# istellartech/OpenGoddard

Hardware: AMD Instinct MI355X
Metric: NLP-callback evals/sec (cost+constr+FD-Jacobian) (higher is better)
Workload: dtype f64; 1 GPU; polar_tsto: 2 phases, [6, 6] states, [3, 3] controls, [80, 80] LGL nodes; n=1442, m_eq=975, m_ineq=640, output_buffers=17 registered persistent-zero replicas of 18.6 MB in rotation, parallelism=fd-columns x1

## Files before the change

opengoddard_amd/csrc/ogk_kernels.hip:

```cpp
#include <hip/hip_runtime.h>
#include "ogk.h"
#include "og_dual.h"
#include OG_GEN_HEADER

typedef double v4f64 __attribute__((ext_vector_type(4)));

#ifndef OGK_EXP
#define OGK_EXP 0
#endif

#ifndef OGK_TRACE
#define OGK_TRACE 0
#endif

namespace {

struct XCol {
    typedef double scalar;
    const double* x0;
    int j;
    double xj;
    __device__ __forceinline__ double operator()(const int i) const {
        const double v = x0[i];
        return i == j ? xj : v;
    }
    __device__ __forceinline__ double ldy(const double* p) const { return *p; }
};

struct XColL {
    typedef double scalar;
    const double* x0;
    int j;
    double xj;
    const double* y0_first;
    const double* yl;
    __device__ __forceinline__ double operator()(const int i) const {
        const double v = x0[i];
        return i == j ? xj : v;
    }
    __device__ __forceinline__ double ldy(const double* p) const { return yl[(int)(p - y0_first)]; }
};

constexpr int TB_SLOTS = OgGen::N_TBLK > 0 ? OgGen::N_TBLK : 1;
struct XColT {
    typedef double scalar;
    const double* x0;
    int j;
    double xj;
    const double* tc;
    int qd[TB_SLOTS];
    double td[TB_SLOTS];
    __device__ __forceinline__ double operator()(const int i) const {
        const double v = x0[i];
        return i == j ? xj : v;
    }
    __device__ __forceinline__ double ldy(const double* p) const { return *p; }
    __device__ __forceinline__ const double* term_cache(const int tb) const {
        return (tc && qd[tb] != -2) ? tc + OgGen::TERM_OFF(tb) : nullptr;
    }
    __device__ __forceinline__ int term_q(const int tb) const { return qd[tb]; }
    __device__ __forceinline__ double term_v(const int tb) const { return td[tb]; }
};
__device__ __forceinline__ XColT make_xcolt(const ogk_args& a, const int j, const double xj, const double* tc) {
    XColT x;
    x.x0 = a.x0, x.j = j, x.xj = xj, x.tc = tc;
    const XCol plain{a.x0, j, xj};
#pragma unroll
    for (int tb = 0; tb < TB_SLOTS; ++tb) {
        x.qd[tb] = -1, x.td[tb] = 0.0;
        if (tc && tb < OgGen::N_TBLK && j >= 0) {
            x.qd[tb] = OgGen::sum_term_q(tb, j);
            if (x.qd[tb] >= 0) x.td[tb] = OgGen::sum_term(tb, x.qd[tb], plain, a.cvec);
        }
    }
    return x;
}
constexpr bool TERM_CACHE = OgGen::N_TERMS > 0 && OgGen::N_TERMS <= 2048;
constexpr int TERM_DOUBLES = TERM_CACHE ? OgGen::N_TERMS + 16 : 0;

template <int THREADS>
__device__ __forceinline__ void fill_terms(const ogk_args& a, double* tc) {
    struct XBase {
        typedef double scalar;
        const double* x0;
        __device__ __forceinline__ double operator()(const int i) const { return x0[i]; }
    };
    const XBase xb{a.x0};
#pragma unroll
    for (int tb = 0; tb < OgGen::N_TBLK; ++tb)
        for (int q = (int)threadIdx.x; q < OgGen::TERM_LEN(tb); q += THREADS)
            tc[OgGen::TERM_OFF(tb) + q] = OgGen::sum_term(tb, q, xb, a.cvec);
}

__device__ __forceinline__ bool jt_needs_fill(const ogk_args& a) {
    const unsigned st = *a.jt_state, gen = *a.jt_launches;
    return !a.jt_sparse | (st == gen - 1u);
}
__device__ __forceinline__ void jt_mark_nan_fill(const ogk_args& a) {
    if (a.jt_sparse) __hip_atomic_store(a.jt_state, *a.jt_launches, __ATOMIC_RELAXED, __HIP_MEMORY_SCOPE_AGENT);
}

constexpr int ROWS_COLS_PER_THREAD = 8;

__device__ __forceinline__ int defect_block_to_group(int bx, int* nt_out) {
    for (int g = 0; g < OgGen::N_GROUPS; ++g) {
        if (OgGen::G_KIND(g) != 1) continue;
        const int ntiles = (OgGen::G_LEN(g) + 15) >> 4;
        if (bx < ntiles) { *nt_out = bx; return g; }
        bx -= ntiles;
    }
    *nt_out = 0;
// ... 284 lines not shown
    const int NP = KS * 4;
    const int tid = (int)threadIdx.x;
    const int wave = tid >> 6, lane = tid & 63, lk = lane >> 4;

    double* dpanel = lds;
    double* xt = lds + KS * 64;
    double* ybuf = xt + OgGen::MAX_NMV * NP;
    const double* src = a.dfrag + a.dfrag_off[rec0.v[5]] + (long)nt * KS * 64;
    constexpr int UNR = 4;
    double pv[UNR];
#pragma unroll
    for (int u = 0; u < UNR; ++u)
        pv[u] = (tid + SWEEP_THREADS * u < KS * 64) ? src[tid + SWEEP_THREADS * u] : 0.0;
    const XCol base{a.x0, -1, 0.0};
    for (int s = wave; s < OgGen::MAX_NMV; s += SWEEP_WAVES)
        for (int l = lane; l < NP; l += 64) {
            double v = 0.0;
            if (s < nmv && l < N) {
                v = OgGen::mv_operand(mv0 + s, l, base, a.cvec);
                if (nt == 0) a.xop[OGT_SLOT[mv0 + s].v[4] + l] = v;
            }
            xt[s * NP + l] = v;
        }
#pragma unroll
    for (int u = 0; u < UNR; ++u)
        if (tid + SWEEP_THREADS * u < KS * 64) dpanel[tid + SWEEP_THREADS * u] = pv[u];
    for (int i = tid + SWEEP_THREADS * UNR; i < KS * 64; i += SWEEP_THREADS) dpanel[i] = src[i];
    __syncthreads();

    constexpr int TR = (OgGen::MAX_NMV + SWEEP_WAVES - 1) / SWEEP_WAVES;
    if (wave == SWEEP_WAVES - 1) {
        const int srow = lane & 15;
        v4f64 acc = {0.0, 0.0, 0.0, 0.0};
        const double* xrow = xt + (srow < OgGen::MAX_NMV ? srow : 0) * NP;
        const bool live = srow < nmv;
        constexpr int CH = 8;
        double bv[CH], av[CH];
#pragma unroll
        for (int u = 0; u < CH; ++u) {
            bv[u] = u < KS ? dpanel[u * 64 + lane] : 0.0;
            av[u] = (u < KS && live) ? xrow[u * 4 + lk] : 0.0;
        }
        for (int ks0 = 0; ks0 < KS; ks0 += CH) {
            double bn[CH], an[CH];
#pragma unroll
            for (int u = 0; u < CH; ++u) {
                const int ks = ks0 + CH + u;
                bn[u] = ks < KS ? dpanel[ks * 64 + lane] : 0.0;
                an[u] = (ks < KS && live) ? xrow[ks * 4 + lk] : 0.0;
            }
#pragma unroll
            for (int u = 0; u < CH; ++u)
                if (ks0 + u < KS) acc = __builtin_amdgcn_mfma_f64_16x16x4f64(av[u], bv[u], acc, 0, 0, 0);
#pragma unroll
            for (int u = 0; u < CH; ++u) { bv[u] = bn[u]; av[u] = an[u]; }
        }
#pragma unroll
        for (int reg = 0; reg < 4; ++reg) ybuf[(lk + 4 * reg) * 16 + (lane & 15)] = acc[reg];
    }
    const int k = nt * 16 + lane;
    const bool node_on = lane < 16 && k < N;
    double T[TR];
#pragma unroll
    for (int r = 0; r < TR; ++r) {
        const int s = wave + r * SWEEP_WAVES;
        T[r] = (node_on && s < nmv) ? OgGen::tail_one(mv0 + s, k, base, a.cvec) : 0.0;
    }
    __syncthreads();
    if (!node_on) return;
#pragma unroll
    for (int r = 0; r < TR; ++r) {
        const int s = wave + r * SWEEP_WAVES;
        if (s >= nmv) break;
        const ogt_int8 rec = OGT_SLOT[mv0 + s];
        const double y = ybuf[s * 16 + lane];
        const int row = rec.v[3] + k;
        publish_row<FUSED>(a, row, y - T[r]);
        a.t0[row] = T[r];
        a.y0[rec.v[4] + k] = y;
    }
}

template <bool FUSED>
__device__ __forceinline__ void eval_rows_body(const ogk_args& a, const int bx, double* lds) {
    bool terms = false;
    if (TERM_CACHE) {
#pragma unroll
        for (int u = 0; u < SWEEP_WAVES; ++u) {
            const int w2 = bx * SWEEP_WAVES + u;
            if (w2 < OGT_N_ROWWAVES) terms = terms || OGT_ROWWAVE[w2].w != 0;
        }
        if (terms) {
            fill_terms<SWEEP_THREADS>(a, lds);
            __syncthreads();
        }
    }
    const int w = bx * SWEEP_WAVES + ((int)threadIdx.x >> 6);
    if (w >= OGT_N_ROWWAVES) return;
    const int4 rw = OGT_ROWWAVE[w];
    const int k = rw.y + ((int)threadIdx.x & 63);
    if (k >= rw.z) return;
    const XColT base = make_xcolt(a, -1, 0.0, terms ? lds : nullptr);
    int row;
    const double v = OgGen::item_value(rw.x, 0, k, base, a.y0, a.cvec, &row);
    publish_row<FUSED>(a, row, v);
}

#ifdef OGK_HAS_MAIN
__global__ __launch_bounds__(SWEEP_THREADS) void ogk_eval(const ogk_args a, const int ndef) {
    extern __shared__ __attribute__((aligned(16))) double lds[];
    const int id = (int)blockIdx.x;
    if (id == 0 && threadIdx.x == 0) {
        *a.nonfinite_next = 0;
        if (a.jt_bump) __hip_atomic_store(a.jt_launches, *a.jt_launches + 1u, __ATOMIC_RELAXED, __HIP_MEMORY_SCOPE_AGENT);
    }
    if (id < ndef) eval_defect_body<false>(a, id, lds);
    else eval_rows_body<false>(a, id - ndef, lds);
}
#endif

#ifndef OGK_LIGHT_COLS
#define OGK_LIGHT_COLS 4
#endif
constexpr int LIGHT_COLS = OGK_LIGHT_COLS;
constexpr int HEAVY_FLAG = 1 << 30;

__device__ __forceinline__ bool marked(const unsigned* bits, const int r) {
    return (bits[r >> 5] >> (r & 31)) & 1u;
}

__device__ __forceinline__ void fill_row(const ogk_args& a, double* jrow, const unsigned* bits,
                                         const int own_lo, const int own_hi, const int first,
                                         const int stride, const bool all_finite,
                                         const bool z_from_this_launch = false) {
    if (OGK_EXP & 16) return;
    if (all_finite) {
        const int a0 = (int)((reinterpret_cast<unsigned long long>(jrow) >> 3) & 1);
        const double2 zero2 = make_double2(0.0, 0.0);
// ... 272 lines not shown
            atomicOr(&bits[r >> 5], 1u << (r & 31));
        }
        __syncthreads();
        fill_row(a, a.jt + (long)(j - a.col_lo) * OgGen::M, bits, own_lo, own_hi, tid, SWEEP_THREADS, false, true);
        __syncthreads();
    }
}

__device__ __forceinline__ void finish_eval(const ogk_args& a, const unsigned n_eval, unsigned* bits) {
    __shared__ int s_last;
    __builtin_amdgcn_s_waitcnt(0);
    __syncthreads();
    if (threadIdx.x == 0) {
        const unsigned t = __hip_atomic_fetch_add(a.ready, 1u, __ATOMIC_RELAXED, __HIP_MEMORY_SCOPE_AGENT);
        int last = 0;
        if (t + 1u == n_eval) {
            const int bad = __hip_atomic_load(a.nonfinite, __ATOMIC_RELAXED, __HIP_MEMORY_SCOPE_AGENT);
            const unsigned st = __hip_atomic_load(a.jt_state, __ATOMIC_RELAXED, __HIP_MEMORY_SCOPE_AGENT);
            const unsigned gen = __hip_atomic_load(a.jt_launches, __ATOMIC_RELAXED, __HIP_MEMORY_SCOPE_AGENT) + 1u;
            __hip_atomic_store(a.ready, 0u, __ATOMIC_RELAXED, __HIP_MEMORY_SCOPE_AGENT);
            __hip_atomic_store(a.jt_launches, gen, __ATOMIC_RELAXED, __HIP_MEMORY_SCOPE_AGENT);
            __hip_atomic_store(a.nonfinite_result, bad, __ATOMIC_RELAXED, __HIP_MEMORY_SCOPE_AGENT);
            if (a.ptail) a.ptail[OgGen::M] = (double)bad;
            __hip_atomic_store(a.nonfinite, 0, __ATOMIC_RELAXED, __HIP_MEMORY_SCOPE_AGENT);
            if (bad != 0) __hip_atomic_store(a.jt_state, gen, __ATOMIC_RELAXED, __HIP_MEMORY_SCOPE_AGENT);
            last = (bad != 0 || st == gen - 1u) ? 1 : 0;
        }
        s_last = last;
    }
    __syncthreads();
    if (s_last) fz_fill_from_z(a, bits);
}

template <class Store>
__device__ __forceinline__ void base_products_tile(const double* panel, const int N, const int nt,
                                                   const int nmv, const double* xt, const int xstride,
                                                   const Store& store) {
    const int lane = (int)threadIdx.x & 63, lk = lane >> 4, srow = lane & 15;
    const int KS = (N + 3) >> 2;
    const double* bsrc = panel + lane;
    const bool live = srow < nmv;
    const double* xrow = xt + (live ? srow : 0) * xstride;
    v4f64 acc = {0.0, 0.0, 0.0, 0.0};
    constexpr int CH = 8;
    double bv[CH], av[CH];
#pragma unroll
    for (int u = 0; u < CH; ++u) {
        const int l = u * 4 + lk;
        bv[u] = u < KS ? bsrc[u * 64] : 0.0;
        av[u] = (u < KS && live && l < N) ? xrow[l] : 0.0;
    }
    for (int ks0 = 0; ks0 < KS; ks0 += CH) {
        double bn[CH], an[CH];
#pragma unroll
        for (int u = 0; u < CH; ++u) {
            const int ks = ks0 + CH + u;
            const int l = ks * 4 + lk;
            bn[u] = ks < KS ? bsrc[ks * 64] : 0.0;
            an[u] = (ks < KS && live && l < N) ? xrow[l] : 0.0;
        }
#pragma unroll
        for (int u = 0; u < CH; ++u)
            if (ks0 + u < KS) acc = __builtin_amdgcn_mfma_f64_16x16x4f64(av[u], bv[u], acc, 0, 0, 0);
#pragma unroll
        for (int u = 0; u < CH; ++u) { bv[u] = bn[u]; av[u] = an[u]; }
    }
    const int k = nt * 16 + (lane & 15);
#pragma unroll
    for (int reg = 0; reg < 4; ++reg) {
        const int st = lk + 4 * reg;
        if (st < nmv && k < N) store(st, k, acc[reg]);
    }
}

constexpr int FZ_COLS = OGT_LGRP_COLS;
template <class XA>
__device__ __forceinline__ void eval_item_paired(const ogk_args& a, const int4 item, const XA& xa, const bool base_role,
                                                 const double dx, double* jrow, double* packed) {
    int row;
    const double v = OgGen::item_value(item.x, item.y, item.z, xa, a.y0, a.cvec, &row);
    const double v0 = __shfl_down(v, FZ_COLS);
    if (!base_role) {
        const double q = (v - v0) / dx;
        jrow[row] = q;
        if (packed) *packed = q;
    }
}

constexpr int FZ_MAXN = OgGen::MAX_NODES;
constexpr int FZ_NP = ((FZ_MAXN + 3) / 4) * 4;
constexpr int FZ_ROUNDS = 2;
constexpr int FZ_ITEM_WAVES = SWEEP_WAVES - 1;
constexpr size_t FZ_TILE_DOUBLES = (size_t)(FZ_NP / 4) * 64 + (size_t)OgGen::MAX_NMV * (FZ_NP + FZ_MAXN);
constexpr size_t FZ_LDS_BYTES = (FZ_TILE_DOUBLES + TERM_DOUBLES) * sizeof(double);

__device__ __forceinline__ void lds_flag_raise(int* flag, const int value) {
    __builtin_amdgcn_fence(__ATOMIC_RELEASE, "workgroup", "local");
    *reinterpret_cast<volatile int*>(flag) = value;
}
__device__ __forceinline__ int lds_flag_wait(int* flag) {
    int v;
    while ((v = *reinterpret_cast<volatile int*>(flag)) == 0) __builtin_amdgcn_s_sleep(1);
    __builtin_amdgcn_fence(__ATOMIC_ACQUIRE, "workgroup", "local");
    return v;
}

#if OGK_TRACE
#define FZ_TRACE_DECL(kind_) long long tr_[6] = {(long long)__builtin_amdgcn_s_memrealtime(), 0, 0, 0, 0, 0}; \
    const int tr_kind_ = (kind_)
#define FZ_STAMP(i) tr_[i] = (long long)__builtin_amdgcn_s_memrealtime()
#define FZ_TRACE_OUT(a_)                                                                                   \
    do {                                                                                                   \
        if (((int)threadIdx.x & 63) == 0 && (a_).trace) {                                                  \
            double* t_ = (a_).trace + ((long)blockIdx.x * SWEEP_WAVES + ((int)threadIdx.x >> 6)) * 8;       \
            t_[0] = (double)tr_kind_; t_[1] = (double)tr_[0]; t_[2] = (double)tr_[1]; t_[3] = (double)tr_[2]; \
            t_[4] = (double)tr_[3]; t_[5] = (double)tr_[4]; t_[6] = (double)tr_[5];                          \
            t_[7] = (double)__builtin_amdgcn_s_memrealtime();                                              \
        }                                                                                                  \
    } while (0)
#else
#define FZ_TRACE_DECL(kind_) do { } while (0)
#define FZ_STAMP(i) do { } while (0)
#define FZ_TRACE_OUT(a_) do { } while (0)
#endif

struct FzTile {
    double* dpanel;
    double* xt;
    double* yb;
};
__device__ __forceinline__ FzTile fz_tile_lds(double* lds) {
    FzTile t;
    t.dpanel = lds;
    t.xt = lds + (FZ_NP / 4) * 64;
    t.yb = t.xt + OgGen::MAX_NMV * FZ_NP;
    return t;
}
__device__ __forceinline__ void fz_stage_tile(const ogk_args& a, const FzTile& t, const int nt, const int mv0,
                                              const int nmv, const int N, const int phase) {
    const int tid = (int)threadIdx.x, lane = tid & 63, wave = tid >> 6;
    const int KS = (N + 3) >> 2, NP = KS << 2;
    constexpr int ST_D = (FZ_NP / 4 * 64 + SWEEP_THREADS - 1) / SWEEP_THREADS;
    constexpr int ST_S = (OgGen::MAX_NMV + SWEEP_WAVES - 1) / SWEEP_WAVES, ST_L = (FZ_NP + 63) / 64;
    const XCol xbase{a.x0, -1, 0.0};
    double st_d[ST_D];
    const double* src = a.dfrag + a.dfrag_off[phase] + (long)nt * KS * 64;
#pragma unroll
    for (int u = 0; u < ST_D; ++u) {
        const int i = tid + u * SWEEP_THREADS;
        st_d[u] = i < KS * 64 ? src[i] : 0.0;
    }
#pragma unroll
    for (int u = 0; u < ST_S; ++u)
#pragma unroll
        for (int q = 0; q < ST_L; ++q) {
            const int sl = wave + u * SWEEP_WAVES, l = lane + q * 64;
            if (sl < nmv && l < NP) t.xt[sl * NP + l] = l < N ? OgGen::mv_operand(mv0 + sl, l, xbase, a.cvec) : 0.0;
        }
#pragma unroll
    for (int u = 0; u < ST_D; ++u) {
        const int i = tid + u * SWEEP_THREADS;
        if (i < KS * 64) t.dpanel[i] = st_d[u];
    }
}

__device__ __forceinline__ void fz_light_body(const ogk_args& a, const int b, double* lds) {
    __shared__ int s_flag;
    FZ_TRACE_DECL(1);
    const ogt_int8 grp = OGT_LGRP[b];
    const int first_j = grp.v[0], cnt = grp.v[1], y0_first = grp.v[2], nt = grp.v[3];
    const int mv0 = grp.v[4], nmv = grp.v[5], N = grp.v[6], phase = grp.v[7] & 0xffff;
    const bool terms = TERM_CACHE && (grp.v[7] >> 16) != 0;
    double* tc = lds + FZ_TILE_DOUBLES;
    const bool has_tile = nmv > 0;
    const int tid = (int)threadIdx.x;
    const int lane = tid & 63, wave = tid >> 6;
    const bool service = wave == SWEEP_WAVES - 1;
    const int cl = lane % FZ_COLS;
    const bool base_role = lane >= FZ_COLS;
    const int ji = first_j + cl;
    const bool item_on = !service && lane < 2 * FZ_COLS && cl < cnt && ji >= a.col_lo && ji < a.col_hi;
    const int4 coli = OGT_LRNG[b * FZ_COLS + cl];
    const double xb = a.x0[item_on ? ji : first_j];
    const double hh = a.h[item_on ? ji : first_j];
    int4 item = make_int4(0, 0, 0, 0);
    const bool has_item = item_on && coli.x + wave < coli.y;
    if (has_item) item = OGT_ELEM[coli.x + wave];

    const FzTile t = fz_tile_lds(lds);
    if (tid == 0) s_flag = 0;
    if (has_tile && !(OGK_FZ & 4)) fz_stage_tile(a, t, nt, mv0, nmv, N, phase);
    if (terms) fill_terms<SWEEP_THREADS>(a, tc);
    lds_barrier();
    FZ_STAMP(1);
    if (service) {
        if (has_tile && !(OGK_FZ & 2))
            base_products_tile(t.dpanel, N, nt, nmv, t.xt, ((N + 3) >> 2) << 2,
                               [&](const int st, const int k, const double v) { t.yb[st * N + k] = v; });
        FZ_STAMP(2);
        if (lane == 0) lds_flag_raise(&s_flag, 1);
        FZ_TRACE_OUT(a);
        return;
    }
    if (has_item && !(OGK_FZ & 2048)) {
        const double xj = xb + hh;
        const double dx = xj - xb;
        double* jrow = a.jt + (long)(ji - a.col_lo) * OgGen::M;
        double* pcol = a.pvals ? a.pvals + a.poff[ji] + (coli.z - coli.x) : nullptr;
        const XColT xa = make_xcolt(a, base_role ? -1 : ji, xj, terms ? tc : nullptr);
        double tv[FZ_ROUNDS];
        int trow[FZ_ROUNDS], tyo[FZ_ROUNDS];
#pragma unroll
        for (int r = 0; r < FZ_ROUNDS; ++r) {
            const int e = coli.x + wave + r * FZ_ITEM_WAVES;
            tv[r] = 0.0, trow[r] = 0, tyo[r] = -1;
            if (e < coli.y) {
                const int4 it = r == 0 ? item : OGT_ELEM[e];
                tv[r] = OgGen::item_tail(it.x, it.y, it.z, xa, a.cvec, &trow[r], &tyo[r]);
            }
        }
        lds_flag_wait(&s_flag);
        FZ_STAMP(3);
#pragma unroll
        for (int r = 0; r < FZ_ROUNDS; ++r) {
            const double v = tyo[r] >= 0 ? t.yb[tyo[r] - y0_first] - tv[r] : tv[r];
            const double v0 = __shfl_down(v, FZ_COLS);
            const int e = coli.x + wave + r * FZ_ITEM_WAVES;
            if (!base_role && e < coli.y) {
                const double q = (v - v0) / dx;
                jrow[trow[r]] = q;
                if (pcol) pcol[e] = q;
            }
        }
        const XColL xl{a.x0, base_role ? -1 : ji, xj, a.y0 + y0_first, t.yb};
        for (int e = coli.x + wave + FZ_ROUNDS * FZ_ITEM_WAVES; e < coli.y; e += FZ_ITEM_WAVES)
            eval_item_paired(a, OGT_ELEM[e], xl, base_role, dx, jrow, pcol ? pcol + e : nullptr);
    }
    FZ_STAMP(4);
    FZ_TRACE_OUT(a);
}

__device__ __forceinline__ void fz_heavy_part(const ogk_args& a, const int pidx, double* lds) {
    __shared__ int s_flag;
    FZ_TRACE_DECL(2);
    const ogt_int8 rec = OGT_HPART[pidx];
    const int j = rec.v[0];
    if (j < a.col_lo || j >= a.col_hi) return;
    const int y0_first = rec.v[3], nt = rec.v[4], mv0 = rec.v[5], nmv = rec.v[6];
    const int N = rec.v[7] & 0xfffff, phase = (rec.v[7] >> 20) & 0x3ff;
    const bool terms = TERM_CACHE && ((rec.v[7] >> 30) & 1) != 0;
    double* tc = lds + FZ_TILE_DOUBLES;
    const bool has_tile = nmv > 0;
    const int tid = (int)threadIdx.x;
    const int lane = tid & 63, wave = tid >> 6;
    const bool service = wave == SWEEP_WAVES - 1;
    const double xb = a.x0[j];
    const double hh = a.h[j];
    const int il = lane & 31;
    const bool base_role = lane >= 32;
    int4 slot = make_int4(0, 0, 0, 0), item = make_int4(0, 0, 0, 0);
    const bool has_slot = !service && rec.v[1] + wave < rec.v[2];
    if (has_slot) {
        slot = OGT_HSLOT[rec.v[1] + wave];
        item = OGT_HELEM[slot.x + (il < slot.y ? il : 0)];
    }
    const FzTile t = fz_tile_lds(lds);
    if (tid == 0) s_flag = 0;
    if (has_tile) fz_stage_tile(a, t, nt, mv0, nmv, N, phase);
    if (terms) fill_terms<SWEEP_THREADS>(a, tc);
    lds_barrier();
    FZ_STAMP(1);
    if (service) {
        if (has_tile)
            base_products_tile(t.dpanel, N, nt, nmv, t.xt, ((N + 3) >> 2) << 2,
                               [&](const int st, const int k, const double v) { t.yb[st * N + k] = v; });
        FZ_STAMP(2);
        if (lane == 0) lds_flag_raise(&s_flag, 1);
        FZ_TRACE_OUT(a);
        return;
    }
    if (has_slot) {
        const double xj = xb + hh;
        const double dx = xj - xb;
        double* jrow = a.jt + (long)(j - a.col_lo) * OgGen::M;
        double* pcol = a.pvals ? a.pvals + a.poff[j] : nullptr;
        const XColT xa = make_xcolt(a, base_role ? -1 : j, xj, terms ? tc : nullptr);
        for (int s0 = rec.v[1] + wave; s0 < rec.v[2]; s0 += FZ_ROUNDS * FZ_ITEM_WAVES) {
            double tv[FZ_ROUNDS];
            int trow[FZ_ROUNDS], tyo[FZ_ROUNDS], cnt[FZ_ROUNDS], tpos[FZ_ROUNDS];
#pragma unroll
            for (int r = 0; r < FZ_ROUNDS; ++r) {
                const int s = s0 + r * FZ_ITEM_WAVES;
                tv[r] = 0.0, trow[r] = 0, tyo[r] = -1, cnt[r] = 0, tpos[r] = 0;
                if (s < rec.v[2]) {
                    const int4 sl = (r == 0 && s0 == rec.v[1] + wave) ? slot : OGT_HSLOT[s];
                    const int4 it = (r == 0 && s0 == rec.v[1] + wave) ? item : OGT_HELEM[sl.x + (il < sl.y ? il : 0)];
                    cnt[r] = sl.y;
                    tpos[r] = it.w;
                    tv[r] = OgGen::item_tail(it.x, it.y, it.z, xa, a.cvec, &trow[r], &tyo[r]);
                }
            }
            if (s0 == rec.v[1] + wave) {
                lds_flag_wait(&s_flag);
                FZ_STAMP(3);
            }
#pragma unroll
            for (int r = 0; r < FZ_ROUNDS; ++r) {
                const double v = tyo[r] >= 0 ? t.yb[tyo[r] - y0_first] - tv[r] : tv[r];
                const double v0 = __shfl_down(v, 32);
                if (!base_role && il < cnt[r]) {
                    const double q = (v - v0) / dx;
                    jrow[trow[r]] = q;
                    if (pcol) pcol[tpos[r]] = q;
                }
            }
        }
    }
    FZ_STAMP(4);
    FZ_TRACE_OUT(a);
}

__device__ __forceinline__ void fz_tile_body(const ogk_args& a, const int bx, double* lds) {
    __shared__ int s_flags[3];
    FZ_TRACE_DECL(3);
    const int4 tile = OGT_FTILE[bx];
    const int slot = tile.x, ct0 = tile.y, nt = tile.z, nct = tile.w;
    const ogt_int8 rec = OGT_SLOT[slot];
    const int N = rec.v[0], leaf = rec.v[2], row0 = rec.v[3];
    const bool diag = rec.v[6] & 1, generic = rec.v[6] & 2;
    const int dep0 = rec.v[7] >> 12, ndep = rec.v[7] & 0xfff;
    const int KS = (N + 3) >> 2;
    const int tid = (int)threadIdx.x;
    const int wave = tid >> 6, lane = tid & 63, lk = lane >> 4, kk = lane & 15;
    double* xt = lds;
    double* yb = lds + FZ_NP;
    double* tb = yb + 16;
    double* td = tb + 16;
    const XCol xbase{a.x0, -1, 0.0};
    for (int l = tid; l < KS * 4; l += SWEEP_THREADS)
        xt[l] = l < N ? OgGen::mv_operand(slot, l, xbase, a.cvec) : 0.0;
    if (tid < 3) s_flags[tid] = 0;
    const int k = nt * 16 + kk;
    const bool k_on = k < N;
    const double* bsrc = a.dfrag + a.dfrag_off[rec.v[5]] + (long)nt * KS * 64 + lane;
    constexpr int CH = 10;
    const int prod_wave = SWEEP_WAVES - 1;
    const int term_wave = nct < SWEEP_WAVES - 1 ? SWEEP_WAVES - 2 : SWEEP_WAVES - 1;
    const bool diag_here = diag && nt >= ct0 && nt < ct0 + nct;
    const int diag_wave = nct < SWEEP_WAVES - 2 ? SWEEP_WAVES - 3 : -1;
    const bool col_wave = wave < nct;
    double bv[CH];
    if (col_wave || wave == prod_wave) {
#pragma unroll
        for (int u = 0; u < CH; ++u) bv[u] = (u < KS) ? bsrc[u * 64] : 0.0;
    }
    lds_barrier();
    FZ_STAMP(1);
    if (!col_wave) {
        if (wave == diag_wave) {
            if (diag_here && lk == 0 && k_on && leaf + k >= a.col_lo && leaf + k < a.col_hi) {
                const int jd = leaf + k;
                const double xbd = a.x0[jd];
                const XCol xd{a.x0, jd, xbd + a.h[jd]};
                td[kk] = OgGen::tail_one(slot, k, xd, a.cvec);
            }
            if (lane == 0) lds_flag_raise(&s_flags[2], 1);
        }
        if (wave == term_wave && lk == 0) tb[kk] = k_on ? OgGen::tail_one(slot, k, xbase, a.cvec) : 0.0;
        if (wave == term_wave && lane == 0) lds_flag_raise(&s_flags[1], 1);
        if (wave == prod_wave) {
                v4f64 accb = {0.0, 0.0, 0.0, 0.0};
            for (int ks0 = 0; ks0 < KS; ks0 += CH) {
                double bn[CH];
#pragma unroll
                for (int u = 0; u < CH; ++u) {
                    const int ks = ks0 + CH + u;
                    bn[u] = (ks < KS) ? bsrc[ks * 64] : 0.0;
                }
#pragma unroll
                for (int u = 0; u < CH; ++u) {
                    const int ks = ks0 + u;
                    if (ks < KS) accb = __builtin_amdgcn_mfma_f64_16x16x4f64(xt[ks * 4 + lk], bv[u], accb, 0, 0, 0);
                }
#pragma unroll
                for (int u = 0; u < CH; ++u) bv[u] = bn[u];
            }
            if (lk == 0) yb[kk] = accb[0];
            FZ_STAMP(2);
            if (lane == 0) lds_flag_raise(&s_flags[0], 1);
        }
        FZ_TRACE_OUT(a);
        return;
    }
    const int l0 = (ct0 + wave) * 16;
    if (l0 >= N || leaf + l0 >= a.col_hi || leaf + l0 + 16 <= a.col_lo) return;
    const int la = l0 + kk;
    const bool a_on = la < N;
    const double xa_b = a.x0[a_on ? leaf + la : leaf];
    const double xa_h = a.h[a_on ? leaf + la : leaf];
    const int row = row0 + (k_on ? k : 0);
    double xbv[4], hv[4];
#pragma unroll
    for (int reg = 0; reg < 4; ++reg) {
        const int lc = l0 + lk + 4 * reg;
        const int jj = leaf + ((k_on && lc < N) ? lc : 0);
        xbv[reg] = a.x0[jj];
        hv[reg] = a.h[jj];
    }
    double t_diag = 0.0;
    bool have_diag = false;
    {
        const int lc = k;
        const int reg = (lc - l0 - lk) >> 2;
        have_diag = diag && k_on && lc >= l0 + lk && ((lc - l0 - lk) & 3) == 0 && reg < 4 && lc < N &&
                    leaf + lc >= a.col_lo && leaf + lc < a.col_hi;
        if (have_diag && diag_wave < 0) {
            const int jd = leaf + lc;
            const double xbd = a.x0[jd];
            const XCol xd{a.x0, jd, xbd + a.h[jd]};
            t_diag = OgGen::tail_one(slot, k, xd, a.cvec);
        }
    }
    double hit_v = 0.0;
    if (a_on) {
        const XCol xa{a.x0, leaf + la, xa_b + xa_h};
        hit_v = OgGen::mv_operand(slot, la, xa, a.cvec);
    }
    v4f64 acc = {0.0, 0.0, 0.0, 0.0};
    for (int ks0 = 0; ks0 < KS; ks0 += CH) {
        double bn[CH];
#pragma unroll
        for (int u = 0; u < CH; ++u) {
            const int ks = ks0 + CH + u;
            bn[u] = (ks < KS) ? bsrc[ks * 64] : 0.0;
        }
#pragma unroll
        for (int u = 0; u < CH; ++u) {
            const int ks = ks0 + u;
            if (ks < KS) {
                const double aop = (ks * 4 + lk == la) ? hit_v : xt[ks * 4 + lk];
                acc = __builtin_amdgcn_mfma_f64_16x16x4f64(aop, bv[u], acc, 0, 0, 0);
            }
        }
#pragma unroll
        for (int u = 0; u < CH; ++u) bv[u] = bn[u];
    }
    FZ_STAMP(2);
    lds_flag_wait(&s_flags[1]);
    lds_flag_wait(&s_flags[0]);
    if (diag_wave >= 0 && l0 == nt * 16) {
        lds_flag_wait(&s_flags[2]);
        if (have_diag) t_diag = td[kk];
    }
    FZ_STAMP(3);
    if (!k_on) return;
    const double t_base = tb[kk];
    const double f_base = yb[kk] - t_base;
#pragma unroll
    for (int reg = 0; reg < 4; ++reg) {
        const int lc = l0 + lk + 4 * reg;
        const int j = leaf + lc;
        if (lc >= N || j < a.col_lo || j >= a.col_hi) continue;
        const double xj = xbv[reg] + hv[reg];
        const double dx = xj - xbv[reg];
        double t = (have_diag && lc == k) ? t_diag : t_base;
        if (generic) {
            bool reads = diag && k == lc;
            for (int d = dep0; d < dep0 + ndep; ++d) {
                const int kind = OgGen::DEP_KIND(d), base_d = OgGen::DEP_BASE(d);
                reads = reads || (kind == 1 ? (base_d + k == j)
                                            : (j >= base_d && j < base_d + OgGen::DEP_CNT(d)));
            }
            if (reads) {
                const XCol xg{a.x0, j, xj};
                t = OgGen::tail_one(slot, k, xg, a.cvec);
            }
        }
        const double val = acc[reg] - t;
        const double q = (val - f_base) / dx;
        a.jt[(long)(j - a.col_lo) * OgGen::M + row] = q;
        if (a.pvals) a.pvals[a.poff[j] + k] = q;
    }
    FZ_STAMP(4);
    FZ_TRACE_OUT(a);
}

#ifndef OGK_FUSED_ATTR
#define OGK_FUSED_ATTR __attribute__((amdgpu_waves_per_eu(4)))
#endif
#ifdef OGK_HAS_FUSED
__global__ __launch_bounds__(SWEEP_THREADS) OGK_FUSED_ATTR void ogk_fused(const ogk_args a, const int ndef, const int n_eval,
                                                           const int group_lo, const int n_light, const int sum_lo,
                                                           const int n_sum) {
    extern __shared__ __attribute__((aligned(16))) double lds[];
    int id = (int)blockIdx.x;
    if (id < n_eval) {
        FZ_TRACE_DECL(0);
        if (!(OGK_FZ & 16)) {
            if (id < ndef) eval_defect_body<true>(a, id, lds);
            else eval_rows_body<true>(a, id - ndef, lds);
        }
        FZ_STAMP(1);
        finish_eval(a, (unsigned)n_eval, reinterpret_cast<unsigned*>(lds));
        FZ_STAMP(4);
        FZ_TRACE_OUT(a);
        return;
    }
    id -= n_eval;
#ifndef OGK_ORDER
#define OGK_ORDER 0
#endif
    const int n_tile = OGT_N_FTILES, n_heavy = OGT_N_HPART;
    int kind, idx;
    if (OGK_ORDER == 0) {
        if (id < n_light) kind = 0, idx = id;
        else if (id < n_light + n_heavy) kind = 1, idx = id - n_light;
        else kind = 2, idx = id - n_light - n_heavy;
// ... 247 lines not shown
```

opengoddard_amd/codegen.py:

```python
from __future__ import annotations

import hashlib

import numpy as np

from . import trace as _tr

import os

HEAVY_COLUMN_ELEMENTS = 32
LIGHT_COLS = 4


def fused_cols(n):
    env = os.environ.get("OG_FUSED_COLS")
    return int(env) if env else 16


def tile_cols():
    env = os.environ.get("OG_TILE_COLS")
    return max(1, min(7, int(env))) if env else 7


MAX_GROUP_OUTPUTS = int(os.environ.get("OG_MAX_GROUP_OUTPUTS", "1"))
# ... 1031 lines not shown
          ",\n".join("    {{%s}}" % ", ".join(str(int(v)) for v in r) for r in (lgrp or [[0] * 8])),
          "};"]
    L += table("int4", "OGT_HSLOT", hslot)
    L += table("int4", "OGT_HELEM", helem)
    L += table("int4", "OGT_LRNG", lrng)
    L += ["static constexpr int OGT_N_LGRP = %d;" % len(light_groups),
          "static const int OGH_LGRP_J[%d] = {%s};" % (len(light_groups) + 1, ", ".join(
              [str(r[0]) for r in light_groups] + [str(P.n)]))]
    with_sum = [i for i, r in enumerate(lgrp) if r[7] & (1 << 16)]
    without = [i for i, r in enumerate(lgrp) if not r[7] & (1 << 16)]
    L += ["static __device__ const int OGT_LSUM[%d] = {%s};" % (max(len(with_sum), 1), ", ".join(map(str, with_sum or [0]))),
          "static __device__ const int OGT_LPLAIN[%d] = {%s};" % (max(len(without), 1), ", ".join(map(str, without or [0]))),
          "static const unsigned char OGH_LGRP_SUM[%d] = {%s};" % (max(len(lgrp), 1), ", ".join(
              "1" if r[7] & (1 << 16) else "0" for r in (lgrp or [[0] * 8])))]
    L += table("int4", "OGT_ROWWAVE", rowwaves)
    L.append("static constexpr int OGT_N_ROWWAVES = %d;" % len(rowwaves))
    L += table("int4", "OGT_COL", col)
    L += table("int4", "OGT_ELEM", elem)
    L += table("int4", "OGT_TILE", tiles)
    ftiles = []
    for si, sl in enumerate(P.mv):
        t16 = (sl.length + 15) // 16
        ngrp = -(-t16 // tile_cols())
        per = -(-t16 // ngrp)
        for c0 in range(0, t16, per):
            for nt in range(t16):
                ftiles.append([si, c0, nt, min(per, t16 - c0)])
    L += table("int4", "OGT_FTILE", ftiles)
    L.append("static constexpr int OGT_N_FTILES = %d;" % len(ftiles))
    L += table("ogt_int8", "OGT_SLOT", [[r] for r in []] or None) if False else \
        ["static __device__ const ogt_int8 OGT_SLOT[%d] = {" % max(len(slots), 1),
         ",\n".join("    {{%s}}" % ", ".join(str(int(v)) for v in r) for r in (slots or [[0] * 8])),
         "};"]
    L += ["static constexpr int OGT_N_TILES = %d;" % len(tiles),
          "static __device__ const int OGT_HEAVY[%d] = {%s};" % (
              max(len(heavy), 1), ", ".join(str(j) for j in heavy) or "0"),
          "#endif", ""]
    return L


def program_hash(source):
    return hashlib.sha256(source.encode()).hexdigest()[:16]
```

Before: 678.9 million callback evals/s.

## Route item tail evaluation through a shared noinline call and pipeline item loops

Item and slot tail evaluations now go through one out-of-line function (item_tail_at, __noinline__ by default) instead of being inlined at every call site via tail_one/item_value. The intent is to shrink code size and register pressure in the fused kernels. The item loops in the two fused column paths are rewritten as a software pipeline: each iteration computes the current tail, prefetches the next element descriptor, and then finishes the previous one. The wait on the staged y tile is deferred until a value that reads y is actually consumed. The risk is call overhead, since ABI register save/restore can slow the hot per-item path. A trace stamp macro is also added.

```diff
diff --git a/opengoddard_amd/csrc/ogk_kernels.hip b/opengoddard_amd/csrc/ogk_kernels.hip
--- a/opengoddard_amd/csrc/ogk_kernels.hip
+++ b/opengoddard_amd/csrc/ogk_kernels.hip
@@ -25,20 +25,6 @@
         return i == j ? xj : v;
     }
     __device__ __forceinline__ double ldy(const double* p) const { return *p; }
-};
-
-struct XColL {
-    typedef double scalar;
-    const double* x0;
-    int j;
-    double xj;
-    const double* y0_first;
-    const double* yl;
-    __device__ __forceinline__ double operator()(const int i) const {
-        const double v = x0[i];
-        return i == j ? xj : v;
-    }
-    __device__ __forceinline__ double ldy(const double* p) const { return yl[(int)(p - y0_first)]; }
 };
 
 constexpr int TB_SLOTS = OgGen::N_TBLK > 0 ? OgGen::N_TBLK : 1;
@@ -77,6 +63,39 @@
 }
 constexpr bool TERM_CACHE = OgGen::N_TERMS > 0 && OgGen::N_TERMS <= 2048;
 constexpr int TERM_DOUBLES = TERM_CACHE ? OgGen::N_TERMS + 16 : 0;
+
+#ifndef OGK_ITEM_CALL
+#define OGK_ITEM_CALL 1
+#endif
+#if OGK_ITEM_CALL
+#define OGK_ITEM_FN __device__ __noinline__
+#else
+#define OGK_ITEM_FN __device__ __forceinline__
+#endif
+struct ItemTail {
+    double v;
+    int row;
+    int yoff;
+};
+OGK_ITEM_FN ItemTail item_tail_at(const int g, const int o, const int k, const double* x0, const int j, const double xj,
+                                  const double* cv) {
+    const XCol x{x0, j, xj};
+    ItemTail r;
+    r.v = OgGen::item_tail(g, o, k, x, cv, &r.row, &r.yoff);
+    return r;
+}
+__device__ __forceinline__ ItemTail item_tail_of(const int4 it, const XColT& x, const double* cv) {
+    if (TERM_CACHE && x.tc) {
+        ItemTail r;
+        r.v = OgGen::item_tail(it.x, it.y, it.z, x, cv, &r.row, &r.yoff);
+        return r;
+    }
+    return item_tail_at(it.x, it.y, it.z, x.x0, x.j, x.xj, cv);
+}
+__device__ __forceinline__ double slot_tail_at(const int slot, const int g, const int k, const double* x0, const int j,
+                                               const double xj, const double* cv) {
+    return item_tail_at(g, slot - OgGen::G_MV0(g), k, x0, j, xj, cv).v;
+}
 
 template <int THREADS>
 __device__ __forceinline__ void fill_terms(const ogk_args& a, double* tc) {
@@ -459,7 +478,7 @@
 #pragma unroll
     for (int r = 0; r < TR; ++r) {
         const int s = wave + r * SWEEP_WAVES;
-        T[r] = (node_on && s < nmv) ? OgGen::tail_one(mv0 + s, k, base, a.cvec) : 0.0;
+        T[r] = (node_on && s < nmv) ? slot_tail_at(mv0 + s, blk.x, k, a.x0, -1, 0.0, a.cvec) : 0.0;
     }
     __syncthreads();
     if (!node_on) return;
@@ -496,9 +515,8 @@
     const int k = rw.y + ((int)threadIdx.x & 63);
     if (k >= rw.z) return;
     const XColT base = make_xcolt(a, -1, 0.0, terms ? lds : nullptr);
-    int row;
-    const double v = OgGen::item_value(rw.x, 0, k, base, a.y0, a.cvec, &row);
-    publish_row<FUSED>(a, row, v);
+    const ItemTail it = item_tail_of(make_int4(rw.x, 0, k, 0), base, a.cvec);
+    publish_row<FUSED>(a, it.row, it.yoff >= 0 ? a.y0[it.yoff] - it.v : it.v);
 }
 
 #ifdef OGK_HAS_MAIN
@@ -879,22 +897,8 @@
 }
 
 constexpr int FZ_COLS = OGT_LGRP_COLS;
-template <class XA>
-__device__ __forceinline__ void eval_item_paired(const ogk_args& a, const int4 item, const XA& xa, const bool base_role,
-                                                 const double dx, double* jrow, double* packed) {
-    int row;
-    const double v = OgGen::item_value(item.x, item.y, item.z, xa, a.y0, a.cvec, &row);
-    const double v0 = __shfl_down(v, FZ_COLS);
-    if (!base_role) {
-        const double q = (v - v0) / dx;
-        jrow[row] = q;
-        if (packed) *packed = q;
-    }
-}
-
 constexpr int FZ_MAXN = OgGen::MAX_NODES;
 constexpr int FZ_NP = ((FZ_MAXN + 3) / 4) * 4;
-constexpr int FZ_ROUNDS = 2;
 constexpr int FZ_ITEM_WAVES = SWEEP_WAVES - 1;
 constexpr size_t FZ_TILE_DOUBLES = (size_t)(FZ_NP / 4) * 64 + (size_t)OgGen::MAX_NMV * (FZ_NP + FZ_MAXN);
 constexpr size_t FZ_LDS_BYTES = (FZ_TILE_DOUBLES + TERM_DOUBLES) * sizeof(double);
@@ -914,6 +918,7 @@
 #define FZ_TRACE_DECL(kind_) long long tr_[6] = {(long long)__builtin_amdgcn_s_memrealtime(), 0, 0, 0, 0, 0}; \
     const int tr_kind_ = (kind_)
 #define FZ_STAMP(i) tr_[i] = (long long)__builtin_amdgcn_s_memrealtime()
+#define FZ_STAMP_LANDED(v) do { asm volatile("" :: "v"(v)); FZ_STAMP(5); } while (0)
 #define FZ_TRACE_OUT(a_)                                                                                   \
     do {                                                                                                   \
         if (((int)threadIdx.x & 63) == 0 && (a_).trace) {                                                  \
@@ -926,6 +931,7 @@
 #else
 #define FZ_TRACE_DECL(kind_) do { } while (0)
 #define FZ_STAMP(i) do { } while (0)
+#define FZ_STAMP_LANDED(v) do { } while (0)
 #define FZ_TRACE_OUT(a_) do { } while (0)
 #endif
 
@@ -991,6 +997,7 @@
     int4 item = make_int4(0, 0, 0, 0);
     const bool has_item = item_on && coli.x + wave < coli.y;
     if (has_item) item = OGT_ELEM[coli.x + wave];
+    FZ_STAMP_LANDED(grp.v[0] + coli.x + item.x);
 
     const FzTile t = fz_tile_lds(lds);
     if (tid == 0) s_flag = 0;
@@ -1013,33 +1020,31 @@
         double* jrow = a.jt + (long)(ji - a.col_lo) * OgGen::M;
         double* pcol = a.pvals ? a.pvals + a.poff[ji] + (coli.z - coli.x) : nullptr;
         const XColT xa = make_xcolt(a, base_role ? -1 : ji, xj, terms ? tc : nullptr);
-        double tv[FZ_ROUNDS];
-        int trow[FZ_ROUNDS], tyo[FZ_ROUNDS];
-#pragma unroll
-        for (int r = 0; r < FZ_ROUNDS; ++r) {
-            const int e = coli.x + wave + r * FZ_ITEM_WAVES;
-            tv[r] = 0.0, trow[r] = 0, tyo[r] = -1;
-            if (e < coli.y) {
-                const int4 it = r == 0 ? item : OGT_ELEM[e];
-                tv[r] = OgGen::item_tail(it.x, it.y, it.z, xa, a.cvec, &trow[r], &tyo[r]);
-            }
-        }
-        lds_flag_wait(&s_flag);
-        FZ_STAMP(3);
-#pragma unroll
-        for (int r = 0; r < FZ_ROUNDS; ++r) {
-            const double v = tyo[r] >= 0 ? t.yb[tyo[r] - y0_first] - tv[r] : tv[r];
-            const double v0 = __shfl_down(v, FZ_COLS);
-            const int e = coli.x + wave + r * FZ_ITEM_WAVES;
-            if (!base_role && e < coli.y) {
-                const double q = (v - v0) / dx;
-                jrow[trow[r]] = q;
-                if (pcol) pcol[e] = q;
-            }
-        }
-        const XColL xl{a.x0, base_role ? -1 : ji, xj, a.y0 + y0_first, t.yb};
-        for (int e = coli.x + wave + FZ_ROUNDS * FZ_ITEM_WAVES; e < coli.y; e += FZ_ITEM_WAVES)
-            eval_item_paired(a, OGT_ELEM[e], xl, base_role, dx, jrow, pcol ? pcol + e : nullptr);
+        ItemTail prev = {0.0, 0, -1};
+        bool seen = false;
+        int4 it = item;
+        for (int e = coli.x + wave; ; e += FZ_ITEM_WAVES) {
+            const bool more = e < coli.y;
+            ItemTail cur = {0.0, 0, -1};
+            if (more) cur = item_tail_of(it, xa, a.cvec);
+            if (e + FZ_ITEM_WAVES < coli.y) it = OGT_ELEM[e + FZ_ITEM_WAVES];
+            if (e != coli.x + wave) {
+                if (prev.yoff >= 0 && !seen) {
+                    lds_flag_wait(&s_flag);
+                    seen = true;
+                    FZ_STAMP(3);
+                }
+                const double v = prev.yoff >= 0 ? t.yb[prev.yoff - y0_first] - prev.v : prev.v;
+                const double v0 = __shfl_down(v, FZ_COLS);
+                if (!base_role) {
+                    const double q = (v - v0) / dx;
+                    jrow[prev.row] = q;
+                    if (pcol) pcol[e - FZ_ITEM_WAVES] = q;
+                }
+            }
+            if (!more) break;
+            prev = cur;
+        }
     }
     FZ_STAMP(4);
     FZ_TRACE_OUT(a);
@@ -1069,6 +1074,7 @@
         slot = OGT_HSLOT[rec.v[1] + wave];
         item = OGT_HELEM[slot.x + (il < slot.y ? il : 0)];
     }
+    FZ_STAMP_LANDED(rec.v[0] + slot.x + item.x);
     const FzTile t = fz_tile_lds(lds);
     if (tid == 0) s_flag = 0;
     if (has_tile) fz_stage_tile(a, t, nt, mv0, nmv, N, phase);
@@ -1090,35 +1096,40 @@
         double* jrow = a.jt + (long)(j - a.col_lo) * OgGen::M;
         double* pcol = a.pvals ? a.pvals + a.poff[j] : nullptr;
         const XColT xa = make_xcolt(a, base_role ? -1 : j, xj, terms ? tc : nullptr);
-        for (int s0 = rec.v[1] + wave; s0 < rec.v[2]; s0 += FZ_ROUNDS * FZ_ITEM_WAVES) {
-            double tv[FZ_ROUNDS];
-            int trow[FZ_ROUNDS], tyo[FZ_ROUNDS], cnt[FZ_ROUNDS], tpos[FZ_ROUNDS];
-#pragma unroll
-            for (int r = 0; r < FZ_ROUNDS; ++r) {
-                const int s = s0 + r * FZ_ITEM_WAVES;
-                tv[r] = 0.0, trow[r] = 0, tyo[r] = -1, cnt[r] = 0, tpos[r] = 0;
-                if (s < rec.v[2]) {
-                    const int4 sl = (r == 0 && s0 == rec.v[1] + wave) ? slot : OGT_HSLOT[s];
-                    const int4 it = (r == 0 && s0 == rec.v[1] + wave) ? item : OGT_HELEM[sl.x + (il < sl.y ? il : 0)];
-                    cnt[r] = sl.y;
-                    tpos[r] = it.w;
-                    tv[r] = OgGen::item_tail(it.x, it.y, it.z, xa, a.cvec, &trow[r], &tyo[r]);
+        const int s_first = rec.v[1] + wave;
+        ItemTail prev = {0.0, 0, -1};
+        int prev_cnt = 0, prev_pos = 0;
+        bool seen = false;
+        int4 sl = slot, it = item;
+        for (int s = s_first; ; s += FZ_ITEM_WAVES) {
+            const bool more = s < rec.v[2];
+            ItemTail cur = {0.0, 0, -1};
+            int cur_cnt = 0, cur_pos = 0;
+            if (more) {
+                cur_cnt = sl.y;
+                cur_pos = it.w;
+                cur = item_tail_of(it, xa, a.cvec);
+            }
+            if (s + FZ_ITEM_WAVES < rec.v[2]) {
+                sl = OGT_HSLOT[s + FZ_ITEM_WAVES];
+                it = OGT_HELEM[sl.x + (il < sl.y ? il : 0)];
+            }
+            if (s != s_first) {
+                if (!seen) {
+                    lds_flag_wait(&s_flag);
+                    seen = true;
+                    FZ_STAMP(3);
                 }
-            }
-            if (s0 == rec.v[1] + wave) {
-                lds_flag_wait(&s_flag);
-                FZ_STAMP(3);
-            }
-#pragma unroll
-            for (int r = 0; r < FZ_ROUNDS; ++r) {
-                const double v = tyo[r] >= 0 ? t.yb[tyo[r] - y0_first] - tv[r] : tv[r];
+                const double v = prev.yoff >= 0 ? t.yb[prev.yoff - y0_first] - prev.v : prev.v;
                 const double v0 = __shfl_down(v, 32);
-                if (!base_role && il < cnt[r]) {
+                if (!base_role && il < prev_cnt) {
                     const double q = (v - v0) / dx;
-                    jrow[trow[r]] = q;
-                    if (pcol) pcol[tpos[r]] = q;
+                    jrow[prev.row] = q;
+                    if (pcol) pcol[prev_pos] = q;
                 }
             }
+            if (!more) break;
+            prev = cur, prev_cnt = cur_cnt, prev_pos = cur_pos;
         }
     }
     FZ_STAMP(4);
@@ -1131,10 +1142,11 @@
     const int4 tile = OGT_FTILE[bx];
     const int slot = tile.x, ct0 = tile.y, nt = tile.z, nct = tile.w;
     const ogt_int8 rec = OGT_SLOT[slot];
-    const int N = rec.v[0], leaf = rec.v[2], row0 = rec.v[3];
+    const int N = rec.v[0], g = rec.v[1], leaf = rec.v[2], row0 = rec.v[3];
     const bool diag = rec.v[6] & 1, generic = rec.v[6] & 2;
     const int dep0 = rec.v[7] >> 12, ndep = rec.v[7] & 0xfff;
     const int KS = (N + 3) >> 2;
+    FZ_STAMP_LANDED(tile.x + N);
     const int tid = (int)threadIdx.x;
     const int wave = tid >> 6, lane = tid & 63, lk = lane >> 4, kk = lane & 15;
     double* xt = lds;
@@ -1166,12 +1178,11 @@
             if (diag_here && lk == 0 && k_on && leaf + k >= a.col_lo && leaf + k < a.col_hi) {
                 const int jd = leaf + k;
                 const double xbd = a.x0[jd];
-                const XCol xd{a.x0, jd, xbd + a.h[jd]};
-                td[kk] = OgGen::tail_one(slot, k, xd, a.cvec);
+                td[kk] = slot_tail_at(slot, g, k, a.x0, jd, xbd + a.h[jd], a.cvec);
             }
             if (lane == 0) lds_flag_raise(&s_flags[2], 1);
         }
-        if (wave == term_wave && lk == 0) tb[kk] = k_on ? OgGen::tail_one(slot, k, xbase, a.cvec) : 0.0;
+        if (wave == term_wave && lk == 0) tb[kk] = k_on ? slot_tail_at(slot, g, k, a.x0, -1, 0.0, a.cvec) : 0.0;
         if (wave == term_wave && lane == 0) lds_flag_raise(&s_flags[1], 1);
         if (wave == prod_wave) {
                 v4f64 accb = {0.0, 0.0, 0.0, 0.0};
@@ -1222,8 +1233,7 @@
         if (have_diag && diag_wave < 0) {
             const int jd = leaf + lc;
             const double xbd = a.x0[jd];
-            const XCol xd{a.x0, jd, xbd + a.h[jd]};
-            t_diag = OgGen::tail_one(slot, k, xd, a.cvec);
+            t_diag = slot_tail_at(slot, g, k, a.x0, jd, xbd + a.h[jd], a.cvec);
         }
     }
     double hit_v = 0.0;
@@ -1276,10 +1286,7 @@
                 reads = reads || (kind == 1 ? (base_d + k == j)
                                             : (j >= base_d && j < base_d + OgGen::DEP_CNT(d)));
             }
-            if (reads) {
-                const XCol xg{a.x0, j, xj};
-                t = OgGen::tail_one(slot, k, xg, a.cvec);
-            }
+            if (reads) t = slot_tail_at(slot, g, k, a.x0, j, xj, a.cvec);
         }
         const double val = acc[reg] - t;
         const double q = (val - f_base) / dx;
```

After: 674.0 million callback evals/s (median of 2 runs). Within noise of the previous version (-0.7%).

## Specialize MFMA K-chains on compile-time depth with full preload and schedule barriers

Applied to the files above, without the earlier changes.

Codegen now emits the set of distinct K-step counts (KS). Kernels dispatch at runtime to a template instantiated for each, and a shared mfma_chain helper fully unrolls the f64 MFMA accumulation. For short chains it preloads every A/B operand into registers before issuing the MFMAs, with sched_barrier fencing to separate loads from math. The aim is to remove loop overhead and runtime bounds predicates and to overlap operand fetch with the MFMA chain. In exchange it raises register pressure from arrays sized KS and adds code-size growth from per-KS instantiation, which may hurt occupancy.

```diff
diff --git a/opengoddard_amd/codegen.py b/opengoddard_amd/codegen.py
--- a/opengoddard_amd/codegen.py
+++ b/opengoddard_amd/codegen.py
@@ -1087,6 +1087,10 @@
         ["static __device__ const ogt_int8 OGT_SLOT[%d] = {" % max(len(slots), 1),
          ",\n".join("    {{%s}}" % ", ".join(str(int(v)) for v in r) for r in (slots or [[0] * 8])),
          "};"]
+    chain_ks = sorted({(sl.length + 3) // 4 for sl in P.mv} |
+                      {(g.length + 3) // 4 for g in P.groups if g.kind == "defect"})
+    L += ["template <int... K> struct OgtKs {};",
+          "using OGT_KS = OgtKs<%s>;" % ", ".join(str(k) for k in chain_ks)]
     L += ["static constexpr int OGT_N_TILES = %d;" % len(tiles),
           "static __device__ const int OGT_HEAVY[%d] = {%s};" % (
               max(len(heavy), 1), ", ".join(str(j) for j in heavy) or "0"),
diff --git a/opengoddard_amd/csrc/ogk_kernels.hip b/opengoddard_amd/csrc/ogk_kernels.hip
--- a/opengoddard_amd/csrc/ogk_kernels.hip
+++ b/opengoddard_amd/csrc/ogk_kernels.hip
@@ -4,6 +4,48 @@
 #include OG_GEN_HEADER
 
 typedef double v4f64 __attribute__((ext_vector_type(4)));
+
+template <int K> struct KsC { static constexpr int value = K; };
+template <class F>
+__device__ __forceinline__ void with_ks(const int, const F&, OgtKs<>) {}
+template <class F, int K0, int... K>
+__device__ __forceinline__ void with_ks(const int ks, const F& f, OgtKs<K0, K...>) {
+    if (ks == K0) f(KsC<K0>());
+    else with_ks(ks, f, OgtKs<K...>());
+}
+
+constexpr int FZ_CHAIN_WHOLE = 20;
+constexpr int FZ_CHAIN_CH = 8;
+struct NoMap {
+    __device__ __forceinline__ double operator()(const int, const double v) const { return v; }
+};
+template <int KS, class Fetch, class AMap = NoMap>
+__device__ __forceinline__ v4f64 mfma_chain(const Fetch& fetch, const AMap& amap = AMap()) {
+    constexpr int CH = KS <= FZ_CHAIN_WHOLE ? KS : FZ_CHAIN_CH;
+    constexpr int NCH = (KS + CH - 1) / CH;
+    double av[KS], bv[KS];
+    v4f64 acc = {0.0, 0.0, 0.0, 0.0};
+#pragma unroll
+    for (int u = 0; u < CH; ++u) fetch(u, av[u], bv[u]);
+    if (NCH == 1) __builtin_amdgcn_s_waitcnt(0xc07f);
+    __builtin_amdgcn_sched_barrier(0);
+#pragma unroll
+    for (int c = 0; c < NCH; ++c) {
+#pragma unroll
+        for (int u = 0; u < CH; ++u) {
+            const int ks = (c + 1) * CH + u;
+            if (ks < KS) fetch(ks, av[ks], bv[ks]);
+        }
+        __builtin_amdgcn_sched_barrier(0);
+#pragma unroll
+        for (int u = 0; u < CH; ++u) {
+            const int ks = c * CH + u;
+            if (ks < KS) acc = __builtin_amdgcn_mfma_f64_16x16x4f64(amap(ks, av[ks]), bv[ks], acc, 0, 0, 0);
+        }
+        __builtin_amdgcn_sched_barrier(0);
+    }
+    return acc;
+}
 
 #ifndef OGK_EXP
 #define OGK_EXP 0
@@ -427,29 +469,14 @@
     if (wave == SWEEP_WAVES - 1) {
         const int srow = lane & 15;
         v4f64 acc = {0.0, 0.0, 0.0, 0.0};
-        const double* xrow = xt + (srow < OgGen::MAX_NMV ? srow : 0) * NP;
-        const bool live = srow < nmv;
-        constexpr int CH = 8;
-        double bv[CH], av[CH];
-#pragma unroll
-        for (int u = 0; u < CH; ++u) {
-            bv[u] = u < KS ? dpanel[u * 64 + lane] : 0.0;
-            av[u] = (u < KS && live) ? xrow[u * 4 + lk] : 0.0;
-        }
-        for (int ks0 = 0; ks0 < KS; ks0 += CH) {
-            double bn[CH], an[CH];
-#pragma unroll
-            for (int u = 0; u < CH; ++u) {
-                const int ks = ks0 + CH + u;
-                bn[u] = ks < KS ? dpanel[ks * 64 + lane] : 0.0;
-                an[u] = (ks < KS && live) ? xrow[ks * 4 + lk] : 0.0;
-            }
-#pragma unroll
-            for (int u = 0; u < CH; ++u)
-                if (ks0 + u < KS) acc = __builtin_amdgcn_mfma_f64_16x16x4f64(av[u], bv[u], acc, 0, 0, 0);
-#pragma unroll
-            for (int u = 0; u < CH; ++u) { bv[u] = bn[u]; av[u] = an[u]; }
-        }
+        const double* xrow = xt + (srow < OgGen::MAX_NMV ? srow : 0) * NP + lk;
+        const double* brow = dpanel + lane;
+        with_ks(KS, [&](auto kc) {
+            acc = mfma_chain<decltype(kc)::value>([&](const int ks, double& av, double& bv) {
+                av = xrow[ks * 4];
+                bv = brow[ks * 64];
+            });
+        }, OGT_KS());
 #pragma unroll
         for (int reg = 0; reg < 4; ++reg) ybuf[(lk + 4 * reg) * 16 + (lane & 15)] = acc[reg];
     }
@@ -837,39 +864,16 @@
     if (s_last) fz_fill_from_z(a, bits);
 }
 
-template <class Store>
+template <int KS, class Store>
 __device__ __forceinline__ void base_products_tile(const double* panel, const int N, const int nt,
-                                                   const int nmv, const double* xt, const int xstride,
-                                                   const Store& store) {
+                                                   const int nmv, const double* xt, const Store& store) {
     const int lane = (int)threadIdx.x & 63, lk = lane >> 4, srow = lane & 15;
-    const int KS = (N + 3) >> 2;
     const double* bsrc = panel + lane;
-    const bool live = srow < nmv;
-    const double* xrow = xt + (live ? srow : 0) * xstride;
-    v4f64 acc = {0.0, 0.0, 0.0, 0.0};
-    constexpr int CH = 8;
-    double bv[CH], av[CH];
-#pragma unroll
-    for (int u = 0; u < CH; ++u) {
-        const int l = u * 4 + lk;
-        bv[u] = u < KS ? bsrc[u * 64] : 0.0;
-        av[u] = (u < KS && live && l < N) ? xrow[l] : 0.0;
-    }
-    for (int ks0 = 0; ks0 < KS; ks0 += CH) {
-        double bn[CH], an[CH];
-#pragma unroll
-        for (int u = 0; u < CH; ++u) {
-            const int ks = ks0 + CH + u;
-            const int l = ks * 4 + lk;
-            bn[u] = ks < KS ? bsrc[ks * 64] : 0.0;
-            an[u] = (ks < KS && live && l < N) ? xrow[l] : 0.0;
-        }
-#pragma unroll
-        for (int u = 0; u < CH; ++u)
-            if (ks0 + u < KS) acc = __builtin_amdgcn_mfma_f64_16x16x4f64(av[u], bv[u], acc, 0, 0, 0);
-#pragma unroll
-        for (int u = 0; u < CH; ++u) { bv[u] = bn[u]; av[u] = an[u]; }
-    }
+    const double* xrow = xt + (srow < nmv ? srow : 0) * (KS * 4) + lk;
+    const v4f64 acc = mfma_chain<KS>([&](const int ks, double& av, double& bv) {
+        av = xrow[ks * 4];
+        bv = bsrc[ks * 64];
+    });
     const int k = nt * 16 + (lane & 15);
 #pragma unroll
     for (int reg = 0; reg < 4; ++reg) {
@@ -1000,8 +1004,10 @@
     FZ_STAMP(1);
     if (service) {
         if (has_tile && !(OGK_FZ & 2))
-            base_products_tile(t.dpanel, N, nt, nmv, t.xt, ((N + 3) >> 2) << 2,
-                               [&](const int st, const int k, const double v) { t.yb[st * N + k] = v; });
+            with_ks((N + 3) >> 2, [&](auto kc) {
+                base_products_tile<decltype(kc)::value>(t.dpanel, N, nt, nmv, t.xt,
+                    [&](const int st, const int k, const double v) { t.yb[st * N + k] = v; });
+            }, OGT_KS());
         FZ_STAMP(2);
         if (lane == 0) lds_flag_raise(&s_flag, 1);
         FZ_TRACE_OUT(a);
@@ -1077,8 +1083,10 @@
     FZ_STAMP(1);
     if (service) {
         if (has_tile)
-            base_products_tile(t.dpanel, N, nt, nmv, t.xt, ((N + 3) >> 2) << 2,
-                               [&](const int st, const int k, const double v) { t.yb[st * N + k] = v; });
+            with_ks((N + 3) >> 2, [&](auto kc) {
+                base_products_tile<decltype(kc)::value>(t.dpanel, N, nt, nmv, t.xt,
+                    [&](const int st, const int k, const double v) { t.yb[st * N + k] = v; });
+            }, OGT_KS());
         FZ_STAMP(2);
         if (lane == 0) lds_flag_raise(&s_flag, 1);
         FZ_TRACE_OUT(a);
@@ -1125,7 +1133,8 @@
     FZ_TRACE_OUT(a);
 }
 
-__device__ __forceinline__ void fz_tile_body(const ogk_args& a, const int bx, double* lds) {
+template <int KS>
+__device__ __forceinline__ void fz_tile_body_k(const ogk_args& a, const int bx, double* lds) {
     __shared__ int s_flags[3];
     FZ_TRACE_DECL(3);
     const int4 tile = OGT_FTILE[bx];
@@ -1134,7 +1143,6 @@
     const int N = rec.v[0], leaf = rec.v[2], row0 = rec.v[3];
     const bool diag = rec.v[6] & 1, generic = rec.v[6] & 2;
     const int dep0 = rec.v[7] >> 12, ndep = rec.v[7] & 0xfff;
-    const int KS = (N + 3) >> 2;
     const int tid = (int)threadIdx.x;
     const int wave = tid >> 6, lane = tid & 63, lk = lane >> 4, kk = lane & 15;
     double* xt = lds;
@@ -1148,17 +1156,21 @@
     const int k = nt * 16 + kk;
     const bool k_on = k < N;
     const double* bsrc = a.dfrag + a.dfrag_off[rec.v[5]] + (long)nt * KS * 64 + lane;
-    constexpr int CH = 10;
+    constexpr int PB = KS <= FZ_CHAIN_WHOLE ? KS : FZ_CHAIN_CH;
     const int prod_wave = SWEEP_WAVES - 1;
     const int term_wave = nct < SWEEP_WAVES - 1 ? SWEEP_WAVES - 2 : SWEEP_WAVES - 1;
     const bool diag_here = diag && nt >= ct0 && nt < ct0 + nct;
     const int diag_wave = nct < SWEEP_WAVES - 2 ? SWEEP_WAVES - 3 : -1;
     const bool col_wave = wave < nct;
-    double bv[CH];
+    double bpre[PB];
     if (col_wave || wave == prod_wave) {
 #pragma unroll
-        for (int u = 0; u < CH; ++u) bv[u] = (u < KS) ? bsrc[u * 64] : 0.0;
-    }
+        for (int u = 0; u < PB; ++u) bpre[u] = bsrc[u * 64];
+    }
+    const auto fetch = [&](const int ks, double& av, double& bv) {
+        av = xt[ks * 4 + lk];
+        bv = ks < PB ? bpre[ks] : bsrc[ks * 64];
+    };
     lds_barrier();
     FZ_STAMP(1);
     if (!col_wave) {
@@ -1174,22 +1186,7 @@
         if (wave == term_wave && lk == 0) tb[kk] = k_on ? OgGen::tail_one(slot, k, xbase, a.cvec) : 0.0;
         if (wave == term_wave && lane == 0) lds_flag_raise(&s_flags[1], 1);
         if (wave == prod_wave) {
-                v4f64 accb = {0.0, 0.0, 0.0, 0.0};
-            for (int ks0 = 0; ks0 < KS; ks0 += CH) {
-                double bn[CH];
-#pragma unroll
-                for (int u = 0; u < CH; ++u) {
-                    const int ks = ks0 + CH + u;
-                    bn[u] = (ks < KS) ? bsrc[ks * 64] : 0.0;
-                }
-#pragma unroll
-                for (int u = 0; u < CH; ++u) {
-                    const int ks = ks0 + u;
-                    if (ks < KS) accb = __builtin_amdgcn_mfma_f64_16x16x4f64(xt[ks * 4 + lk], bv[u], accb, 0, 0, 0);
-                }
-#pragma unroll
-                for (int u = 0; u < CH; ++u) bv[u] = bn[u];
-            }
+            const v4f64 accb = mfma_chain<KS>(fetch);
             if (lk == 0) yb[kk] = accb[0];
             FZ_STAMP(2);
             if (lane == 0) lds_flag_raise(&s_flags[0], 1);
@@ -1231,25 +1228,9 @@
         const XCol xa{a.x0, leaf + la, xa_b + xa_h};
         hit_v = OgGen::mv_operand(slot, la, xa, a.cvec);
     }
-    v4f64 acc = {0.0, 0.0, 0.0, 0.0};
-    for (int ks0 = 0; ks0 < KS; ks0 += CH) {
-        double bn[CH];
-#pragma unroll
-        for (int u = 0; u < CH; ++u) {
-            const int ks = ks0 + CH + u;
-            bn[u] = (ks < KS) ? bsrc[ks * 64] : 0.0;
-        }
-#pragma unroll
-        for (int u = 0; u < CH; ++u) {
-            const int ks = ks0 + u;
-            if (ks < KS) {
-                const double aop = (ks * 4 + lk == la) ? hit_v : xt[ks * 4 + lk];
-                acc = __builtin_amdgcn_mfma_f64_16x16x4f64(aop, bv[u], acc, 0, 0, 0);
-            }
-        }
-#pragma unroll
-        for (int u = 0; u < CH; ++u) bv[u] = bn[u];
-    }
+    const v4f64 acc = mfma_chain<KS>(fetch, [&](const int ks, const double v) {
+        return ks * 4 + lk == la ? hit_v : v;
+    });
     FZ_STAMP(2);
     lds_flag_wait(&s_flags[1]);
     lds_flag_wait(&s_flags[0]);
@@ -1288,6 +1269,10 @@
     }
     FZ_STAMP(4);
     FZ_TRACE_OUT(a);
+}
+__device__ __forceinline__ void fz_tile_body(const ogk_args& a, const int bx, double* lds) {
+    const int KS = (OGT_SLOT[OGT_FTILE[bx].x].v[0] + 3) >> 2;
+    with_ks(KS, [&](auto kc) { fz_tile_body_k<decltype(kc)::value>(a, bx, lds); }, OGT_KS());
 }
 
 #ifndef OGK_FUSED_ATTR
```

Result: slower. 677.2 million callback evals/s before, 666.4 million callback evals/s after, median of 2 (-1.6%).
